# sid2364/dna-sequences-pg-extension

Hardware: AMD Instinct MI355X
Metric: k-mers/sec for k=31 count over 3 Gbase synthetic; % of HBM-read roofline (higher is better)
Workload: dtype u64; 1 GPU; config 4: k=31 count over 3000000000 synthetic bases (splitmix64 seed 0xd2a0003), unordered groups (super-k-mer partitioning), single GPU; n_bases=3000000000, k=31, distinct=2999999968

## Files before the change

dna-sequences-pg-extension_amd/csrc/kernels.hpp:

```cpp
#pragma once
#include <hip/hip_runtime.h>
#include <stdint.h>

#include "kmer_device.hpp"

namespace dnagpu {

hipError_t launch_synth(u64 *words, u64 w_begin, u64 w_end, u64 n_bases, u64 seed, u64 motif_len, hipStream_t s);
hipError_t launch_extract(const u64 *words, u64 n_words, u64 first, u64 count, int k, u64 *out_keys,
                          hipStream_t s);

constexpr int FILTER_MAX_GROUPS = 8192;
struct FilterSource {
    const u64 *words;
    u64 n_words;
    const u32 *marks;
    u64 n_mark_words;
    const u64 *seq_starts;
    u64 n_seqs;
};
void filter_bits_geometry(u64 count, u32 *n_groups, u32 *tiles_per_group);
hipError_t launch_filter_bits_count(const FilterSource &src, u64 first, u64 count, const FilterBits &fb, u32 *group_counts,
                                    hipStream_t s);
hipError_t launch_filter_bits_write(const FilterSource &src, u64 first, u64 count, const FilterBits &fb,
// ... 151 lines not shown
hipError_t launch_query_rank_scatter(const QHistSrc &s, u32 n_classes, u64 *cursors, u64 *out_keys, u64 *out_counts, u64 rows,
                                     hipStream_t st);
hipError_t launch_query_rank_scatter(const QAccSrc &s, u32 n_classes, u64 *cursors, u64 *out_keys, u64 *out_counts, u64 rows,
                                     hipStream_t st);
hipError_t launch_query_reverse(u64 *keys, u64 *counts, u64 n, hipStream_t st);

hipError_t launch_batch_marks(const u64 *starts, u64 n_seqs, u32 *marks, u64 n_mark_words, hipStream_t s);
hipError_t launch_batch_rows(const u64 *starts, u64 n_seqs, int k, u64 *rows, hipStream_t s);
hipError_t launch_batch_keys(const u64 *words, u64 n_words, const u32 *marks, u64 n_mark_words, u64 n_rows, int k, u64 *out_keys,
                             unsigned long long *cursor, hipStream_t s);

int sk_min_k();
int sk_minimizer_len(int k);
int sk_tile_rows();
int sk_max_c0();
hipError_t launch_sk_level0(bool scatter, const Chunk *chunks, u32 n_chunks, const u64 *words, u64 n_words, u64 first, int k,
                            u32 c0n, u32 b1bits, u32 r0bits, u32 *hist, const u32 *tot, void *recs, hipStream_t s,
                            u32 *aux = nullptr, const u32 *marks = nullptr, u64 n_mark_words = 0);
hipError_t launch_sk_sample_chunks(Chunk *chunks, u32 n_chunks, u32 stride, u32 len, u32 n, hipStream_t s);
int sk_slab_words();
u32 sk_slab_cap(u32 est, u64 chunk_rows, u64 sampled);
hipError_t launch_sk_slab_init(const u32 *est, u32 r0bits, u32 chunk_rows, u32 sampled, u32 n_chunks, u32 *slab, Node *nodes,
                               hipStream_t s);
hipError_t launch_sk_hist1(const Node *nodes, const Chunk *chunks, u32 n_chunks, const void *recs, u32 *hist, u32 *kcount,
                           hipStream_t s, bool by_d2 = false);
hipError_t launch_sk_scatter1(const Node *nodes, const Chunk *chunks, u32 n_chunks, const void *src, void *dst, const u32 *hist,
                              const u32 *tot, hipStream_t s, bool by_d2 = false, u32 *gcur = nullptr);
u64 sk_spec_span(u32 len, int bits);
hipError_t launch_sk_spec_regions(const Node *nodes, u32 n_nodes, u32 *spec, u32 *out, u32 *gcur, hipStream_t s,
                                  const u32 *rstart = nullptr);
hipError_t launch_sk_scatter1_spec(const Node *nodes, const Chunk *chunks, u32 n_chunks, const void *src, void *dst, u32 *gcur,
                                   const u32 *spec, u32 *kcount, u32 *over, hipStream_t s, const u32 *rstart = nullptr,
                                   const u32 *rcap = nullptr);
hipError_t launch_sk_spec_nodes(const Node *nodes, u32 n_nodes, const u32 *spec, const u32 *gcur, Node *next, u32 *over,
                                hipStream_t s, const u32 *rstart = nullptr, const u32 *rcap = nullptr);
u32 sk_sample1_len();
u32 sk_sample1_every();
hipError_t launch_sk_sampled_regions(const Node *nodes, const Chunk *samples, u32 n_samples, const void *recs, u32 n_mid, u32 *est,
                                     u32 *rcap, u32 *rstart, u32 *scan_tmp, u32 *total, hipStream_t s);
hipError_t launch_sk_heavy_finals(const Node *kids, u32 n, const u32 *kcount, Node *out, hipStream_t s);
int sk_flat_slice();
hipError_t launch_sk_take_heavy(Node *mids, const u32 *idx, u32 n_heavy, const u32 *kcount, Node *out, hipStream_t s);
hipError_t launch_sk_slice_count(const Node *buckets, u32 nb, u32 *n_slices, hipStream_t s);
hipError_t launch_sk_slice_fill(const Node *buckets, u32 nb, const u32 *slice_first, u32 *slice_rec0, u32 *slice_nrec, hipStream_t s);
hipError_t launch_sk_slice_kmers(const void *recs, const u32 *slice_rec0, const u32 *slice_nrec, u32 n_slices, u32 *slice_km,
                                 hipStream_t s);
hipError_t launch_sk_slice_nodes(const Node *buckets, u32 nb, const u32 *slice_first, const u32 *slice_koff, u32 n_slices,
                                 const u32 *total_keys, u32 key_base, int k, bool check_kmers, Node *out, u64 *n_bad, hipStream_t s);
hipError_t launch_sk_unmix(u64 *keys, u64 first, const u64 *end, u64 max_groups, int k, hipStream_t s);
hipError_t launch_sk_expand_flat(const void *recs, const u32 *slice_rec0, const u32 *slice_nrec, const u32 *slice_koff, u32 key_base,
                                 u32 n_slices, int k, u64 *keys, hipStream_t s);
int sk_regroup_tile();
hipError_t launch_sk_regroup(const Node *mids, u32 n_mids, const void *src, void *dst, Node *out_nodes, bool any_long, hipStream_t s);
hipError_t launch_sk_count(const Node *fin, const u32 *list, const u32 *list_off, u32 n_list, const void *recs, int k, u64 *n_groups,
                           u64 *seg_off, u32 *seg_cnt, u64 *out_keys, u32 *out_counts, u32 *left, hipStream_t s);

int sk_count_cap();
hipError_t launch_sk_select_flags(const Node *fin, u32 n_fin, u32 cap, u32 big_limit, u32 *f_small, u32 *f_big, u32 *k_range,
                                  u32 *k_big, hipStream_t s);
hipError_t launch_sk_select_lists(const Node *fin, u32 n_fin, u32 cap, u32 big_limit, const u32 *p_small, const u32 *p_big,
                                  const u32 *kb_range, u32 *list_small, u32 *off_small, u32 *list_big, u32 *off_big, hipStream_t s);
hipError_t launch_sk_over_flags(const Node *fin, u32 n_fin, u32 cap, u32 big_limit, const u32 *p_big, const u32 *big_status,
                                u32 *f_over, u32 *k_over, hipStream_t s);
hipError_t launch_sk_over_list(const Node *fin, u32 n_fin, const u32 *f_raw, const u32 *p_over, const u32 *kb_over, Node *over_nodes,
                               u32 *over_kbase, hipStream_t s);
hipError_t launch_sk_node_lens(const Node *nodes, u32 n, u32 *lens, hipStream_t s);
u32 sk_big_slice_records();
u64 sk_big_partial_slots();
hipError_t launch_sk_big_slices(const Node *fin, const u32 *list, u32 n_list, u32 *nsl, u32 *msl, hipStream_t s);
hipError_t launch_sk_big_slice_fill(const u32 *nsl_raw, const u32 *sfirst, u32 n_list, u32 *sl_bucket, u32 *sl_idx, hipStream_t s);
hipError_t launch_sk_count_big(const Node *fin, const u32 *list, const u32 *list_off, const u32 *nsl, const u32 *mfirst,
                               const u32 *sl_bucket, const u32 *sl_idx, u32 n_slices, u32 n_list, const void *recs, int k,
                               u64 *n_groups, u64 *seg_off, u32 *seg_cnt, u64 *out_keys, u32 *out_counts, u32 *status, u64 *part_keys,
                               u32 *part_cnts, u32 *part_n, bool any_sliced, hipStream_t s);

int scatter_tile_keys();
int scatter_threads();

}
```

dna-sequences-pg-extension_amd/csrc/sk_host.hip:

```cpp
#include "host_common.hpp"

using namespace dnagpu;


constexpr u64 SK_LEAF_MEAN = 2500;
constexpr u64 SK_MID_LIMIT = (u64)1 << 27;
#ifndef SK_MID_RECORDS_LOG2
#define SK_MID_RECORDS_LOG2 16
#endif
constexpr u32 SK_MID_RECORDS = 1u << SK_MID_RECORDS_LOG2;
constexpr u64 SK_BIG_LIMIT = 0xFFFFFFFFull;
constexpr int SK_B1_MAX = 9;
constexpr u64 SK_SLAB_MIN_ROWS = (u64)1 << 29;

template <typename T>
static int alloc1(PoolScope &ps, size_t n, T **out, size_t per = 1)
{
    return ps.alloc(std::max<size_t>(n, 1) * per, out);
}

static u32 sk_chunk_len(u64 x, u64 target = 4096, u64 tile = 8192)
{
    const u64 len = std::max<u64>(4 * tile, (x + target - 1) / target);
    return (u32)((len + tile - 1) / tile * tile);
// ... 476 lines not shown
    HIP_TRY(launch_level_children(hnodes, nh, lh.tot, lh.next, nullptr, nullptr, nullptr, 0, st));
    HIP_TRY(launch_sk_scatter1(hnodes, lh.chunks, lh.n_chunks, l1.rec1, p.rec0, lh.hist, lh.tot, st, true));
    p.heavy.total = 0;
    return DNAGPU_OK;
}

static int sk_level2(dnagpu_ctx *ctx, PoolScope &ps, SkParts &p, SkL1 &l1, const SkSplit &split)
{
    hipStream_t st = ctx->stream;
    const u32 n_mid = l1.lv.n_next, n_split = split.lv.n_next;
    Node *fn = nullptr;
    RC_TRY(ps.alloc((size_t)n_mid * 16 + n_split, &fn));
    prof_mark(ctx, "sk_regroup");
    bool any_long = false;
    for (u32 i = 0; i < n_mid && !any_long; i++)
        any_long = l1.rcn[i] > (u32)sk_regroup_tile();
    HIP_TRY(launch_sk_regroup(l1.lv.next, n_mid, l1.rec1, p.rec0, fn, any_long, st));
    if (n_split)
        HIP_TRY(launch_sk_heavy_finals(split.lv.next, n_split, split.kcount, fn + (size_t)n_mid * 16, st));
    if (!l1.rec1_kept)
        ps.free_now(l1.rec1);
    p.recs = p.rec0;
    p.fin = fn;
    p.n_fin = n_mid * 16 + n_split;
    return DNAGPU_OK;
}

static int sk_levels12(dnagpu_ctx *ctx, PoolScope &ps, SkParts &p)
{
    SkL1 l1;
    SkL1Route route;
    RC_TRY(sk_l1_plan(ctx, ps, p, l1));
    RC_TRY(sk_l1_route(ctx, ps, p, l1, &route));
    bool moved = false;
    if (route != SkL1Route::Exact)
        RC_TRY(sk_l1_speculative(ctx, ps, p, l1, route, &moved));
    if (!moved)
        RC_TRY(sk_l1_histogram(ctx, p, l1));
    std::vector<u32> heavy_idx;
    RC_TRY(sk_l1_census(ctx->debug_flags, l1, p, &heavy_idx));
    if (!moved)
        RC_TRY(sk_l1_scatter(ctx, ps, p, l1));
    SkSplit split;
    if (!heavy_idx.empty())
        RC_TRY(sk_heavy_take(ctx, ps, p, l1, heavy_idx, &split));
    return sk_level2(ctx, ps, p, l1, split);
}


struct SkTail {
    u32 *f_small = nullptr, *f_big = nullptr, *k_range = nullptr, *f_over = nullptr;
    u32 *scan_tmp = nullptr, *totals = nullptr;
    u32 *list_small = nullptr, *off_small = nullptr, *list_big = nullptr, *off_big = nullptr;
    u32 n_small = 0, n_big = 0, big_kmers = 0;
    u64 small_keys = 0;
    u64 out_cap = 0;
    u64 *cursor = nullptr;
    u64 *ok = nullptr;
    u32 *oc = nullptr;
    u64 *seg_off_fin = nullptr;
    u32 *seg_cnt_fin = nullptr;
    u32 *big_status = nullptr;
    Node *over_nodes = nullptr;
    u32 n_over = 0;
    u64 over_keys = 0;
    TreeResult tr = {};
    u64 *seg_off = nullptr;
    u32 *seg_cnt = nullptr;
    u32 n_segs = 0;
};

static int sk_tail_select(dnagpu_ctx *ctx, PoolScope &ps, const SkParts &p, u64 n, SkTail &t)
{
    hipStream_t st = ctx->stream;
    const u32 n_fin = p.n_fin;
    prof_mark(ctx, "sk_select");
    RC_TRY(ps.alloc((size_t)n_fin, &t.f_small));
    RC_TRY(ps.alloc((size_t)n_fin, &t.f_big));
    RC_TRY(ps.alloc((size_t)n_fin, &t.k_range));
    RC_TRY(ps.alloc((size_t)scan_tmp_words(n_fin) * 4, &t.scan_tmp));
    RC_TRY(ps.alloc(8, &t.totals));
    RC_TRY(ps.alloc((size_t)n_fin, &t.list_small));
    RC_TRY(ps.alloc((size_t)n_fin, &t.off_small));
    RC_TRY(ps.alloc((size_t)n_fin, &t.f_over));
    HIP_TRY(launch_sk_select_flags(p.fin, n_fin, (u32)sk_count_cap(), (u32)SK_BIG_LIMIT, t.f_small, t.f_big, t.k_range, t.f_over, st));
    HIP_TRY(launch_scan_u32_multi(scans_in_place({t.f_small, t.f_big, t.k_range, t.f_over}, t.totals, t.scan_tmp), 4, n_fin, st));
    u32 ht[4] = {0, 0, 0, 0};
    RC_TRY(read_back(ctx, ht, t.totals, sizeof ht));
    t.n_small = ht[0];
    t.n_big = ht[1];
    t.small_keys = ht[2];
    t.big_kmers = ht[3];
    t.out_cap = n + t.big_kmers;
    RC_TRY(alloc1(ps, t.n_big, &t.list_big));
    RC_TRY(alloc1(ps, t.n_big, &t.off_big));
    HIP_TRY(launch_sk_select_lists(p.fin, n_fin, (u32)sk_count_cap(), (u32)SK_BIG_LIMIT, t.f_small, t.f_big, t.k_range, t.list_small,
                                   t.off_small, t.list_big, t.off_big, st));
    return DNAGPU_OK;
}

static int sk_tail_outputs(dnagpu_ctx *ctx, PoolScope &ps, const SkParts &p, SkTail &t)
{
    hipStream_t st = ctx->stream;
    const u32 n_fin = p.n_fin;
    RC_TRY(ps.alloc(3, &t.cursor));
    RC_TRY(ps.alloc((size_t)t.out_cap, &t.ok));
    RC_TRY(ps.alloc((size_t)t.out_cap, &t.oc));
    const u64 init[3] = {t.small_keys, 0, 0};
    HIP_TRY(poke(t.cursor, init, sizeof init, st));
    RC_TRY(alloc1(ps, n_fin, &t.seg_off_fin));
    RC_TRY(alloc1(ps, n_fin, &t.seg_cnt_fin));
    HIP_TRY(hipMemsetAsync(t.seg_cnt_fin, 0, (size_t)n_fin * sizeof(u32), st));
    HIP_TRY(hipMemsetAsync(t.seg_off_fin, 0, (size_t)n_fin * sizeof(u64), st));
    RC_TRY(alloc1(ps, t.n_big, &t.big_status));
    return DNAGPU_OK;
}

static int sk_tail_count_big(dnagpu_ctx *ctx, PoolScope &ps, const SkParts &p, SkTail &t)
{
    hipStream_t st = ctx->stream;
    const u32 n_big = t.n_big;
    prof_mark(ctx, "sk_count_big");
    u32 *nsl = nullptr, *sfirst = nullptr, *mfirst = nullptr, *sl_bucket = nullptr, *sl_idx = nullptr, *part_n = nullptr, *part_cnts = nullptr;
    u64 *part_keys = nullptr;
    RC_TRY(ps.alloc((size_t)n_big, &nsl));
    RC_TRY(ps.alloc((size_t)n_big, &sfirst));
    RC_TRY(ps.alloc((size_t)n_big, &mfirst));
    HIP_TRY(launch_sk_big_slices(p.fin, t.list_big, n_big, nsl, mfirst, st));
    HIP_TRY(launch_scan_u32(nsl, sfirst, n_big, t.scan_tmp, t.totals + 6, st));
    HIP_TRY(launch_scan_u32(mfirst, mfirst, n_big, t.scan_tmp, t.totals + 7, st));
    u32 hs[2] = {0, 0};
    RC_TRY(read_back(ctx, hs, t.totals + 6, sizeof hs));
    const u32 n_slices = hs[0], n_part = hs[1];
    RC_TRY(alloc1(ps, n_slices, &sl_bucket));
    RC_TRY(alloc1(ps, n_slices, &sl_idx));
    RC_TRY(alloc1(ps, n_part, &part_n));
    RC_TRY(alloc1(ps, n_part, &part_keys, sk_big_partial_slots()));
    RC_TRY(alloc1(ps, n_part, &part_cnts, sk_big_partial_slots()));
    HIP_TRY(launch_sk_big_slice_fill(nsl, sfirst, n_big, sl_bucket, sl_idx, st));
    HIP_TRY(launch_sk_count_big(p.fin, t.list_big, t.off_big, nsl, mfirst, sl_bucket, sl_idx, n_slices, n_big, p.recs, p.k, t.cursor + 2,
                                t.seg_off_fin, t.seg_cnt_fin, t.ok, t.oc, t.big_status, part_keys, part_cnts, part_n, n_part > 0, st));
    return DNAGPU_OK;
}

static int sk_tail_select_over(dnagpu_ctx *ctx, PoolScope &ps, const SkParts &p, SkTail &t)
{
    hipStream_t st = ctx->stream;
    const u32 n_fin = p.n_fin;
    u32 *f_over_raw = nullptr, *k_over = nullptr, *over_kbase = nullptr;
    prof_mark(ctx, "sk_select_over");
// ... 43 lines not shown
        const u64 tree_keys = t.over_keys + heavy.total;
        if (tree_keys > 0xFFFFFFFFull)
            return DNAGPU_ERR_TOO_LARGE;
        const u32 n_tree = t.n_over + heavy.n;
        u64 *kbuf = nullptr;
        Node *knodes = nullptr;
        RC_TRY(ps.alloc((size_t)tree_keys, &kbuf));
        RC_TRY(ps.alloc((size_t)n_tree, &knodes));
        prof_mark(ctx, "sk_expand_flat");
        if (t.n_over)
            RC_TRY(sk_tail_expand(ctx, ps, t, p.k, t.over_nodes, t.n_over, p.recs, 0, true, kbuf, knodes));
        if (heavy.n)
            RC_TRY(sk_tail_expand(ctx, ps, t, p.k, heavy.nodes, heavy.n, heavy.recs, (u32)t.over_keys, heavy.counted, kbuf,
                                  knodes + t.n_over));
        RC_TRY(run_tree(ctx, ps, nullptr, 0, tree_keys, p.k, kbuf, 0, &t.tr, 0, 0, true, 0, ~0u, 0, knodes, n_tree, 2));
    }
#ifdef DNAGPU_STAMPS
    fprintf(stderr, "[sk select] n_fin %u small %u big %u (k-mers of big %u) over %u (keys %llu) heavy %u (keys %llu) tree nodes %u tiny %u small %u big %u\n",
            p.n_fin, t.n_small, t.n_big, t.big_kmers, t.n_over, (unsigned long long)t.over_keys, heavy.n,
            (unsigned long long)heavy.total, t.tr.n_nodes, t.tr.n_tiny, t.tr.n_small, t.tr.n_big);
#endif
    return DNAGPU_OK;
}

static int sk_tail_leaves(dnagpu_ctx *ctx, PoolScope &ps, const SkParts &p, SkTail &t)
{
    hipStream_t st = ctx->stream;
    const u32 n_fin = p.n_fin;
    const TreeResult &tr = t.tr;
    t.n_segs = n_fin + tr.n_nodes;
    RC_TRY(ps.alloc((size_t)t.n_segs, &t.seg_off));
    RC_TRY(ps.alloc((size_t)t.n_segs, &t.seg_cnt));
    HIP_TRY(hipMemcpyAsync(t.seg_cnt, t.seg_cnt_fin, (size_t)n_fin * sizeof(u32), hipMemcpyDeviceToDevice, st));
    HIP_TRY(hipMemcpyAsync(t.seg_off, t.seg_off_fin, (size_t)n_fin * sizeof(u64), hipMemcpyDeviceToDevice, st));
    if (tr.n_nodes > 0) {
        u32 *flags = nullptr, *ltmp = nullptr, *cls_list = nullptr;
        RC_TRY(ps.alloc((size_t)tr.n_nodes + 1, &flags));
        RC_TRY(ps.alloc((size_t)scan_tmp_words(tr.n_nodes), &ltmp));
        RC_TRY(ps.alloc((size_t)tr.n_nodes, &cls_list));
        prof_mark(ctx, "leaves");
        HIP_TRY(launch_leaves(tr.nodes, tr.n_nodes, tr.n_tiny, tr.n_small, tr.n_big, tr.buf0, tr.buf1, t.cursor, t.seg_off + n_fin,
                              t.seg_cnt + n_fin, t.ok, t.oc, flags, ltmp, cls_list, st, true, t.small_keys));
        HIP_TRY(launch_sk_unmix(t.ok, t.small_keys, t.cursor, tr.n_keys, p.k, st));
    }
    return DNAGPU_OK;
}

static int sk_tail_count(dnagpu_ctx *ctx, PoolScope &ps, const SkParts &p, SkTail &t)
{
    hipStream_t st = ctx->stream;
    prof_mark(ctx, "sk_count");
    u32 *left = nullptr;
    RC_TRY(ps.alloc((size_t)2 * t.n_small + 1, &left));
    HIP_TRY(launch_sk_count(p.fin, t.list_small, t.off_small, t.n_small, p.recs, p.k, t.cursor + 2, t.seg_off, t.seg_cnt, t.ok, t.oc, left,
                            st));
#ifdef DNAGPU_STAMPS
    {
        u32 nl = 0;
        RC_TRY(read_back(ctx, &nl, left + 2 * (size_t)t.n_small, 4));
        fprintf(stderr, "[sk count] %u small buckets, %u left to sk_count by sk_count_clean\n", t.n_small, nl);
    }
#endif
    return DNAGPU_OK;
}

static int sk_tail_finish(dnagpu_ctx *ctx, PoolScope &ps, const SkTail &t, u64 n, dnagpu_hist *h)
{
    prof_mark(ctx, "end");
    u64 fin_ctr[3] = {0, 0, 0};
    RC_TRY(read_back(ctx, fin_ctr, t.cursor, 24));
    const u64 extent = fin_ctr[0];
    const u64 total_groups = fin_ctr[2] + (extent - t.small_keys);
    if (fin_ctr[1] != 0) {
        set_err("super-k-mer count: %llu buckets whose records expand to a different number of k-mers than the partition counted",
                (unsigned long long)fin_ctr[1]);
        return DNAGPU_ERR_INTERNAL;
    }
    if (extent > t.out_cap) {
        set_err("super-k-mer count: %llu output slots used, %llu allocated", (unsigned long long)extent, (unsigned long long)t.out_cap);
        return DNAGPU_ERR_INTERNAL;
    }
    if (total_groups > n) {
        set_err("super-k-mer count: %llu groups for %llu rows", (unsigned long long)total_groups, (unsigned long long)n);
        return DNAGPU_ERR_INTERNAL;
    }
    h->total = n;
    hist_adopt(ps, h, t.ok, t.oc, t.seg_off, t.seg_cnt, t.n_segs, total_groups, false, extent);
    return DNAGPU_OK;
}

static int count_sk_tail(dnagpu_ctx *ctx, PoolScope &ps, const SkParts &p, u64 n, dnagpu_hist *h)
{
    SkTail t;
    RC_TRY(sk_tail_select(ctx, ps, p, n, t));
    RC_TRY(sk_tail_outputs(ctx, ps, p, t));
    if (t.n_big)
        RC_TRY(sk_tail_count_big(ctx, ps, p, t));
    RC_TRY(sk_tail_select_over(ctx, ps, p, t));
    RC_TRY(sk_tail_tree(ctx, ps, p, t));
    RC_TRY(sk_tail_leaves(ctx, ps, p, t));
    RC_TRY(sk_tail_count(ctx, ps, p, t));
    return sk_tail_finish(ctx, ps, t, n, h);
}

int dnagpu::count_sk(dnagpu_ctx *ctx, const SkRows &rows, int k, dnagpu_hist *h, u64 n_kmers_expected)
{
    PoolScope ps(ctx);
    SkParts p;
// ... 186 lines not shown
```

dna-sequences-pg-extension_amd/csrc/superkmer_kernels.hip:

```cpp
#include <algorithm>
#include <cstdlib>
#include <type_traits>

#include "kernels.hpp"

namespace dnagpu {

constexpr int SK_NT = 256;
constexpr int SKW_ROWS = 63 * 32;
constexpr int SK_TILE_ROWS = (SK_NT / 64) * SKW_ROWS;
constexpr int SK_MAX_C0 = 256;
constexpr int SKW_LIST = 768;
__host__ __device__ constexpr u32 sk_plain_max(int w) { return (u32)(2 * SKW_ROWS * 17 / (10 * (w + 1))) < (u32)SKW_LIST ? (u32)(2 * SKW_ROWS * 17 / (10 * (w + 1))) : (u32)SKW_LIST; }

int sk_tile_rows() { return SK_TILE_ROWS; }
int sk_max_c0() { return SK_MAX_C0; }
int sk_count_cap() { return 4096; }

typedef unsigned long long ull2_t __attribute__((ext_vector_type(2)));

constexpr int SK_REC_MULTI_BIT = 58;
constexpr int SK_POS_SHIFT = 39;
constexpr u32 SK_POS_MASK = 31u;
constexpr u32 SK_GPOS_MASK = 63u;
// ... 1740 lines not shown
                    ownq[q0 + q] = (unsigned short)((u32)tid | (q << 9));
            }
            myrec.x = myrec.y = 0;
            if (has_next2 && (u32)tid < nn2.len)
                myrec = recs[(u64)nn2.start + tid];
        }
        lq += step;
        li = ln;
        off = off_next;
        nd = nn;
        has_next = has_next2;
        ln = ln2;
        off_next = off2;
        nn = nn2;
    }
    emit_prev();
    if (tid == 0)
        atomicAdd(n_groups, (unsigned long long)my_groups);
}

__device__ __forceinline__ bool sk_records_share_kmer(const ull2_t A, u32 a, u32 nba, const ull2_t B, u32 b, u32 nbb, u32 m, u32 kmm)
{
    const u64 pm = ((u64)1 << 34) - 1;
    const u64 ah = A.y & pm, bh = B.y & pm;
    const u32 ML = a < b ? a : b;
    const u32 ra = nba - a - m, rb = nbb - b - m;
    const u32 MR = ra < rb ? ra : rb;
    const u64 xr = (sk_shr128(A.x, ah, 2u * (a + m)) ^ sk_shr128(B.x, bh, 2u * (b + m))) & (((u64)1 << (2u * MR)) - 1);
    const u32 R = xr ? (u32)__builtin_ctzll(xr) >> 1 : MR;
    if (R + ML < kmm)
        return false;
    const u64 xl = (funnel(A.x, ah, 2u * (a - ML)) ^ funnel(B.x, bh, 2u * (b - ML))) & (((u64)1 << (2u * ML)) - 1);
    const u32 L = xl ? ML - 1u - ((63u - (u32)__builtin_clzll(xl)) >> 1) : ML;
    return L + R >= kmm;
}


constexpr int SKQ_NT = 512;
static_assert(SKQ_NT == SKC_MAXREC, "a thread per record");
constexpr int SKQ_KMERS = 4096;
constexpr int SKQ_VSLOTS = 1024;
constexpr int SKQ_DIRTY_MAX = 640;

#if defined(SKQ_STORE_PLAIN) || defined(SKQ_KEYS_PLAIN)
#define SKQ_STORE(v, p) (*(p) = (v))
#else
#define SKQ_STORE(v, p) __builtin_nontemporal_store(v, p)
#endif
#if defined(SKQ_STORE_PLAIN) || defined(SKQ_COUNTS_PLAIN)
#define SKQ_STOREC(v, p) (*(p) = (v))
#else
#define SKQ_STOREC(v, p) __builtin_nontemporal_store(v, p)
#endif
__global__ __launch_bounds__(SKQ_NT, 8) void sk_count_clean_kernel(const Node *__restrict__ fin, const u32 *__restrict__ list,
                                                                   const u32 *__restrict__ list_off, u32 n_list,
                                                                   const ull2_t *__restrict__ recs, int k,
                                                                   unsigned long long *__restrict__ n_groups,
                                                                   u64 *__restrict__ seg_off, u32 *__restrict__ seg_cnt,
                                                                   u64 *__restrict__ out_keys, u32 *__restrict__ out_counts,
                                                                   u32 *__restrict__ left_list, u32 *__restrict__ left_off,
                                                                   u32 *__restrict__ n_left, int dbg)
{
    constexpr int WAVES = SKQ_NT / 64;
    __shared__ __attribute__((aligned(16))) ull2_t lrec[SKC_MAXREC];
    __shared__ __attribute__((aligned(16))) u64 vtab[SKQ_VSLOTS];
    __shared__ unsigned short own[SKQ_KMERS];
    __shared__ u32 wk[WAVES], wk2[WAVES];
    __shared__ u32 shared_flag[2], multi_flag[2];
    __shared__ u32 dcnt2[SKQ_VSLOTS / 2];
    __shared__ unsigned short cpos[SKC_MAXREC];
    __shared__ unsigned char rdb[SKC_MAXREC];
    __shared__ u32 d_ones;
    unsigned short *dcnt = reinterpret_cast<unsigned short *>(dcnt2);
    int tid = threadIdx.x;
    u32 lq = blockIdx.x;
    if (lq >= n_list)
        return;
    vtab[tid] = ~(u64)0;
    vtab[tid + SKQ_NT] = ~(u64)0;
    dcnt2[tid] = 0;
    rdb[tid] = 0;
    if (tid < 2)
        shared_flag[tid] = multi_flag[tid] = 0;
    if (tid == 0)
        d_ones = 0;
    const u32 mlen = k >= 23 ? 15u : (k >= 21 ? 13u : 12u);
    const u32 vmask = (1u << (2u * mlen)) - 1u, kmm = (u32)k - mlen;
    const u32 flank = kmm / 2u < 8u ? kmm / 2u : 8u, fmask = (1u << (2u * flank)) - 1u;
    const u32 hmask = (u32)(kmer_mask(k) >> 32);
    const u32 step = gridDim.x;
    u32 li = list[lq];
    Node nd = fin[li];
    ull2_t myrec;
    myrec.x = myrec.y = 0;
    if ((u32)tid < nd.len)
        myrec = recs[(u64)nd.start + tid];
    u64 my_groups = 0;
    int par = 0;
    for (;;) {
        const u32 off = list_off[lq];
        const bool has_next = lq + step < n_list;
        const u32 ln = has_next ? list[lq + step] : li;
        const Node nn = fin[ln];
        asm volatile("" : "+v"(tid));
        const int lane = tid & 63, wave = tid >> 6;
        const ull2_t me = myrec;
        lrec[tid] = me;
        myrec.x = myrec.y = 0;
        if (has_next && (u32)tid < nn.len)
            myrec = recs[(u64)nn.start + tid];
        const bool have = (u32)tid < nd.len;
        const u32 yh = (u32)(me.y >> 32);
        const u32 len = have ? ((yh >> 12) & 31u) + 1u : 0u;
        const u32 kinc = wave_incl_scan(len);
        if (lane == 63)
            wk[wave] = kinc;
        __syncthreads();
        u32 kbase = 0, n_km = 0;
        sk_wave_prefix16(wk, WAVES, wave, lane, kbase, n_km);
        u32 vslot = ~0u;
        if (have) {
            const u32 k0 = kbase + kinc - len;
            if (!SK_DBG(1024))
                for (u32 j = 0; j < len; j++)
                    own[k0 + j] = (unsigned short)((u32)tid | (j << 9));
            if (SK_DBG(256)) {
            } else if (yh & (1u << (SK_REC_MULTI_BIT - 32))) {
                multi_flag[par] = 1u;
            } else {
                const u32 p0 = (u32)me.x, p1 = (u32)(me.x >> 32), p2 = (u32)me.y, p3 = yh & 3u;
                const u32 a = (yh >> (SK_POS_SHIFT - 32)) & SK_POS_MASK;
                const u32 nba = len + (u32)k - 1u;
                const u32 sv = 2u * a, sl = 2u * (a - flank), sr = 2u * (a + mlen);
                const u32 v = __builtin_amdgcn_alignbit(sv >= 32u ? p2 : p1, sv >= 32u ? p1 : p0, sv) & vmask;
                u32 fl = __builtin_amdgcn_alignbit(sl >= 32u ? p2 : p1, sl >= 32u ? p1 : p0, sl) & fmask;
                const u32 r_lo = sr >= 64u ? p2 : (sr >= 32u ? p1 : p0), r_hi = sr >= 64u ? p3 : (sr >= 32u ? p2 : p1);
                u32 fr = __builtin_amdgcn_alignbit(r_hi, r_lo, sr) & fmask;
                const u32 mine_own = 0x8000u | (u32)tid;
                fl = a >= flank ? fl : mine_own;
                fr = nba - a - mlen >= flank ? fr : mine_own;
                const u32 hv = (v ^ (v >> 13)) * 0x85EBCA6Bu;
                const u32 lo32 = (hv >> 10) | ((u32)tid << 22), hi32 = fl | (fr << 16);
                const u64 mine = (u64)lo32 | ((u64)hi32 << 32);
                u32 slot = hv >> 22;
                for (;;) {
                    const u64 old = atomicCAS(reinterpret_cast<unsigned long long *>(&vtab[slot]), ~0ull, (unsigned long long)mine);
                    if (old == ~(u64)0)
                        break;
                    const u32 xl = (u32)old ^ lo32, xh = (u32)(old >> 32) ^ hi32;
                    if ((xl & 0x3FFFFFu) == 0 && ((xh & 0xFFFFu) == 0 || (xh >> 16) == 0)) {
                        const u32 oid = ((u32)old >> 22) & 511u;
                        const ull2_t ot = lrec[oid];
                        const u32 oyh = (u32)(ot.y >> 32);
                        if (sk_records_share_kmer(me, a, nba, ot, (oyh >> (SK_POS_SHIFT - 32)) & SK_POS_MASK,
                                                  ((oyh >> 12) & 31u) + (u32)k, mlen, kmm)) {
                            shared_flag[par] = 1u;
                            rdb[tid] = 1;
                            rdb[oid] = 1;
                        }
                    }
                    slot = (slot + 1u) & (u32)(SKQ_VSLOTS - 1);
                }
                vslot = slot;
            }
        }
        __syncthreads();
        if (vslot != ~0u)
            vtab[vslot] = ~(u64)0;
        u64 *ok = out_keys + off;
        u32 *oc = out_counts + off;
        auto key_cut = [&](const ull2_t r, u32 e) -> u64 {
            const u32 p0 = (u32)r.x, p1 = (u32)(r.x >> 32), p2 = (u32)r.y, p3 = (u32)(r.y >> 32) & 3u;
            const u32 sh = 2u * (e >> 9);
            const bool up = sh >= 32u;
            const u32 a0 = up ? p1 : p0, a1 = up ? p2 : p1, a2 = up ? p3 : p2;
            const u32 kl = __builtin_amdgcn_alignbit(a1, a0, sh), kh = __builtin_amdgcn_alignbit(a2, a1, sh) & hmask;
            return ((u64)kh << 32) | kl;
        };
        auto key_of = [&](u32 i) -> u64 {
            const u32 e = own[i];
            return key_cut(lrec[e & 511u], e);
        };
        const u32 flag = shared_flag[par] | (multi_flag[par] << 1);
        if (flag) {
            const bool dirty = have && rdb[tid] != 0;
            rdb[tid] = 0;
            const u32 pk = dirty ? (len << 16) : len;
            const u32 pinc = wave_incl_scan(pk);
            if (lane == 63)
                wk2[wave] = pinc;
            __syncthreads();
            u32 pbase = 0, ptot = 0;
            sk_wave_prefix16(wk2, WAVES, wave, lane, pbase, ptot);
            const u32 n_clean = ptot & 0xFFFFu, n_dirty = ptot >> 16;
            if ((flag & 2u) || n_dirty > (u32)SKQ_DIRTY_MAX) {
                if (tid == 0) {
                    const u32 d = atomicAdd(n_left, 1u);
                    left_list[d] = li;
                    left_off[d] = off;
                }
            } else {
                cpos[tid] = dirty ? (unsigned short)0xFFFFu : (unsigned short)((pbase + pinc - pk) & 0xFFFFu);
                __syncthreads();
                for (u32 i = (u32)tid; i < n_km; i += SKQ_NT) {
                    const u32 e = own[i];
                    const u32 c = cpos[e & 511u];
                    const u64 key = key_of(i);
                    if (c != 0xFFFFu) {
                        SKQ_STORE(key, &ok[c + (e >> 9)]);
                        SKQ_STOREC(1u, &oc[c + (e >> 9)]);
                    } else if (key == ~(u64)0) {
                        atomicAdd(&d_ones, 1u);
                    } else {
                        u32 slot = ((((u32)key ^ (u32)(key >> 32)) * 0x9E3779B1u) >> 22) & (u32)(SKQ_VSLOTS - 1);
                        for (;;) {
                            const u64 old = atomicCAS(reinterpret_cast<unsigned long long *>(&vtab[slot]), ~0ull, (unsigned long long)key);
                            if (old == ~(u64)0 || old == key)
                                break;
                            slot = (slot + 1u) & (u32)(SKQ_VSLOTS - 1);
                        }
                        atomicAdd(&dcnt2[slot >> 1], 1u << ((slot & 1u) * 16u));
// ... 43 lines not shown
            if ((u32)tid < head && (u32)tid < n_km) {
                SKQ_STORE(key_of((u32)tid), &ok[tid]);
                SKQ_STOREC(1u, &oc[tid]);
            }
            u32 i = head + 2u * (u32)tid;
            u32 e0 = 0, e1 = 0;
            ull2_t r0, r1;
            r0.x = r0.y = r1.x = r1.y = 0;
            auto fetch = [&](u32 at) {
                e0 = own[at];
                e1 = own[at + 1 < n_km ? at + 1 : at];
                asm volatile("" : "+v"(e0), "+v"(e1));
                r0 = lrec[e0 & 511u];
                r1 = lrec[e1 & 511u];
                asm volatile("" : "+v"(r0.x), "+v"(r0.y), "+v"(r1.x), "+v"(r1.y));
            };
            if (i < n_km)
                fetch(i);
            while (i < n_km) {
                const u32 ce0 = e0, ce1 = e1;
                const ull2_t c0 = r0, c1 = r1;
                const u32 nxt = i + 2u * SKQ_NT;
                if (nxt < n_km)
                    fetch(nxt);
                const u64 k0 = key_cut(c0, ce0);
                if (SK_DBG(512)) {
                    if (k0 == 0x123456789ull)
                        ok[0] = k0;
                } else if (i + 1 < n_km) {
                    ull2_t kk;
                    kk.x = k0;
                    kk.y = key_cut(c1, ce1);
                    SKQ_STORE(kk, reinterpret_cast<ull2_t *>(&ok[i]));
                    SKQ_STOREC((u64)0x100000001ull, reinterpret_cast<u64 *>(&oc[i]));
                } else {
                    SKQ_STORE(k0, &ok[i]);
                    SKQ_STOREC(1u, &oc[i]);
                }
                i = nxt;
            }
            if (tid == 0) {
                seg_off[li] = off;
                seg_cnt[li] = n_km;
                my_groups += n_km;
            }
        }
        if (tid == 0)
            shared_flag[par ^ 1] = multi_flag[par ^ 1] = 0;
        par ^= 1;
        if (!has_next)
            break;
        __syncthreads();
        lq += step;
        li = ln;
        nd = nn;
    }
    if (tid == 0 && my_groups)
        atomicAdd(n_groups, (unsigned long long)my_groups);
}

static int sk_dbg();

hipError_t launch_sk_count(const Node *fin, const u32 *list, const u32 *list_off, u32 n_list, const void *recs, int k, u64 *n_groups,
                           u64 *seg_off, u32 *seg_cnt, u64 *out_keys, u32 *out_counts, u32 *left ,
                           hipStream_t s)
{
    if (n_list == 0)
        return hipSuccess;
    int dev = 0, n_cu = 256, v = 0;
    if (hipGetDevice(&dev) == hipSuccess && hipDeviceGetAttribute(&v, hipDeviceAttributeMultiprocessorCount, dev) == hipSuccess && v > 0)
        n_cu = v;
    u32 *left_list = left, *left_off = left + n_list, *n_left = left + 2 * (size_t)n_list;
    hipError_t e = hipMemsetAsync(n_left, 0, sizeof(u32), s);
    if (e != hipSuccess)
        return e;
    hipLaunchKernelGGL(sk_count_clean_kernel, dim3(std::min<u32>(n_list, (u32)n_cu * 4u)), dim3(SKQ_NT), 0, s, fin, list, list_off, n_list,
                       reinterpret_cast<const ull2_t *>(recs), k, reinterpret_cast<unsigned long long *>(n_groups), seg_off, seg_cnt,
                       out_keys, out_counts, left_list, left_off, n_left, sk_dbg());
    const u32 grid = std::min<u32>(n_list, (u32)n_cu * 2u);
    hipLaunchKernelGGL(sk_count_kernel, dim3(grid), dim3(SKC_NT), 0, s, fin, left_list, left_off, 0u, n_left,
                       reinterpret_cast<const ull2_t *>(recs), k, reinterpret_cast<unsigned long long *>(n_groups), seg_off, seg_cnt,
                       out_keys, out_counts, sk_dbg());
    return hipGetLastError();
}

constexpr int SKB_NT = 1024;
constexpr int SKB_SLOTS = 8192;
constexpr int SKB_REC = 512;
constexpr int SKB_MAXQ = SKB_REC * 8;
constexpr u32 SKB_ROUND_CAP = SKB_SLOTS - SKB_NT * SKC_KPT - 64;
constexpr u64 SKB_EMPTY = ~(u64)0;
constexpr int SKB_RTAB_BITS = 10;
static_assert((1 << SKB_RTAB_BITS) == SKB_NT, "one record-table slot per thread");

__device__ __forceinline__ u32 skb_emit(const u64 *tab, const u32 *cnt, u32 n_ones, u32 *wtot, u64 *dst_keys, u32 *dst_counts)
{
    constexpr int WAVES = SKB_NT / 64;
    const int tid = threadIdx.x, lane = tid & 63, wave = tid >> 6;
    u64 myk[8];
    u32 myc[8], mine = 0;
#pragma unroll
    for (int j = 0; j < 8; j++) {
        myk[j] = tab[tid * 8 + j];
        myc[j] = cnt[tid * 8 + j];
        mine += myk[j] != SKB_EMPTY ? 1u : 0u;
    }
    const u32 inc = wave_incl_scan(mine);
    if (lane == 63)
        wtot[wave] = inc;
    __syncthreads();
    u32 before = 0, D = 0;
    sk_wave_prefix16(wtot, WAVES, wave, lane, before, D);
    u64 o = before + inc - mine;
#pragma unroll
    for (int j = 0; j < 8; j++)
        if (myk[j] != SKB_EMPTY) {
            dst_keys[o] = myk[j];
            dst_counts[o] = myc[j];
            o++;
        }
    if (n_ones && tid == 0) {
        dst_keys[D] = SKB_EMPTY;
        dst_counts[D] = n_ones;
    }
    return D + (n_ones ? 1u : 0u);
}

constexpr u32 SKB_SLICE_REC = 128 * SKB_REC;
constexpr u32 SKB_FAILED = ~0u;
// ... 322 lines not shown
        return hipSuccess;
    hipLaunchKernelGGL(sk_big_slice_fill_kernel, dim3((n_list + 3) / 4), dim3(256), 0, s, nsl_raw, sfirst, n_list, sl_bucket, sl_idx);
    return hipGetLastError();
}

hipError_t launch_sk_count_big(const Node *fin, const u32 *list, const u32 *list_off, const u32 *nsl, const u32 *mfirst,
                               const u32 *sl_bucket, const u32 *sl_idx, u32 n_slices, u32 n_list, const void *recs, int k,
                               u64 *n_groups, u64 *seg_off, u32 *seg_cnt, u64 *out_keys, u32 *out_counts, u32 *status, u64 *part_keys,
                               u32 *part_cnts, u32 *part_n, bool any_sliced, hipStream_t s)
{
    if (n_slices == 0)
        return hipSuccess;
    int dev = 0, n_cu = 256, v = 0;
    if (hipGetDevice(&dev) == hipSuccess && hipDeviceGetAttribute(&v, hipDeviceAttributeMultiprocessorCount, dev) == hipSuccess && v > 0)
        n_cu = v;
    const u32 grid = std::min<u32>(n_slices, (u32)n_cu);
    hipLaunchKernelGGL(sk_count_big_kernel, dim3(grid), dim3(SKB_NT), 0, s, fin, list, list_off, nsl, mfirst, sl_bucket, sl_idx,
                       n_slices, reinterpret_cast<const ull2_t *>(recs), k, reinterpret_cast<unsigned long long *>(n_groups), seg_off,
                       seg_cnt, out_keys, out_counts, status, part_keys, part_cnts, part_n);
    if (any_sliced)
        hipLaunchKernelGGL(sk_big_merge_kernel, dim3(n_list), dim3(SKB_NT), 0, s, fin, list, list_off, nsl, mfirst, n_list,
                           reinterpret_cast<unsigned long long *>(n_groups), seg_off, seg_cnt, out_keys, out_counts, status,
                           part_keys, part_cnts, part_n);
    return hipGetLastError();
}

__device__ __forceinline__ u32 sk_bucket_class(const Node &nd, u32 cap, u32 big_limit)
{
    const u32 km = nd.child_base;
    if (km == 0)
        return 0u;
    if (km <= cap && nd.len <= (u32)SKC_MAXREC && nd.chunk_base <= (u32)SKC_MAXQ)
        return 1u;
    return km > 2 * cap && km <= big_limit ? 2u : 3u;
}

__global__ __launch_bounds__(256) void sk_select_flags_kernel(const Node *__restrict__ fin, u32 n_fin, u32 cap, u32 big_limit,
                                                              u32 *__restrict__ f_small, u32 *__restrict__ f_big,
                                                              u32 *__restrict__ k_range, u32 *__restrict__ k_big)
{
    const u32 i = blockIdx.x * blockDim.x + threadIdx.x;
    if (i >= n_fin)
        return;
    const u32 c = sk_bucket_class(fin[i], cap, big_limit);
    f_small[i] = c == 1u ? 1u : 0u;
    f_big[i] = c == 2u ? 1u : 0u;
    k_range[i] = c == 1u || c == 2u ? fin[i].child_base : 0u;
    k_big[i] = c == 2u ? fin[i].child_base : 0u;
}

__global__ __launch_bounds__(256) void sk_select_lists_kernel(const Node *__restrict__ fin, u32 n_fin, u32 cap, u32 big_limit,
                                                              const u32 *__restrict__ p_small, const u32 *__restrict__ p_big,
                                                              const u32 *__restrict__ kb_range, u32 *__restrict__ list_small,
                                                              u32 *__restrict__ off_small, u32 *__restrict__ list_big,
                                                              u32 *__restrict__ off_big)
{
    const u32 i = blockIdx.x * blockDim.x + threadIdx.x;
    if (i >= n_fin)
        return;
    const u32 c = sk_bucket_class(fin[i], cap, big_limit);
    if (c == 1u) {
        list_small[p_small[i]] = i;
        off_small[p_small[i]] = kb_range[i];
    } else if (c == 2u) {
        list_big[p_big[i]] = i;
        off_big[p_big[i]] = kb_range[i];
    }
}

__global__ __launch_bounds__(256) void sk_over_flags_kernel(const Node *__restrict__ fin, u32 n_fin, u32 cap, u32 big_limit,
                                                            const u32 *__restrict__ p_big, const u32 *__restrict__ big_status,
                                                            u32 *__restrict__ f_over, u32 *__restrict__ k_over)
{
    const u32 i = blockIdx.x * blockDim.x + threadIdx.x;
    if (i >= n_fin)
        return;
    const u32 c = sk_bucket_class(fin[i], cap, big_limit);
    const bool over = c == 3u || (c == 2u && big_status[p_big[i]] != 0);
    f_over[i] = over ? 1u : 0u;
    k_over[i] = over ? fin[i].child_base : 0u;
}

__global__ __launch_bounds__(256) void sk_over_list_kernel(const Node *__restrict__ fin, u32 n_fin, const u32 *__restrict__ f_raw,
                                                           const u32 *__restrict__ p_over, const u32 *__restrict__ kb_over,
                                                           Node *__restrict__ over_nodes, u32 *__restrict__ over_kbase)
{
    const u32 i = blockIdx.x * blockDim.x + threadIdx.x;
    if (i >= n_fin || !f_raw[i])
        return;
    over_nodes[p_over[i]] = fin[i];
    over_kbase[p_over[i]] = kb_over[i];
}

hipError_t launch_sk_select_flags(const Node *fin, u32 n_fin, u32 cap, u32 big_limit, u32 *f_small, u32 *f_big, u32 *k_range,
                                  u32 *k_big, hipStream_t s)
{
    if (n_fin == 0)
        return hipSuccess;
    hipLaunchKernelGGL(sk_select_flags_kernel, dim3((n_fin + 255) / 256), dim3(256), 0, s, fin, n_fin, cap, big_limit, f_small, f_big,
                       k_range, k_big);
    return hipGetLastError();
}

hipError_t launch_sk_select_lists(const Node *fin, u32 n_fin, u32 cap, u32 big_limit, const u32 *p_small, const u32 *p_big,
                                  const u32 *kb_range, u32 *list_small, u32 *off_small, u32 *list_big, u32 *off_big, hipStream_t s)
{
    if (n_fin == 0)
        return hipSuccess;
    hipLaunchKernelGGL(sk_select_lists_kernel, dim3((n_fin + 255) / 256), dim3(256), 0, s, fin, n_fin, cap, big_limit, p_small, p_big,
                       kb_range, list_small, off_small, list_big, off_big);
    return hipGetLastError();
}

hipError_t launch_sk_over_flags(const Node *fin, u32 n_fin, u32 cap, u32 big_limit, const u32 *p_big, const u32 *big_status,
                                u32 *f_over, u32 *k_over, hipStream_t s)
{
    if (n_fin == 0)
        return hipSuccess;
    hipLaunchKernelGGL(sk_over_flags_kernel, dim3((n_fin + 255) / 256), dim3(256), 0, s, fin, n_fin, cap, big_limit, p_big, big_status,
                       f_over, k_over);
    return hipGetLastError();
}

hipError_t launch_sk_over_list(const Node *fin, u32 n_fin, const u32 *f_raw, const u32 *p_over, const u32 *kb_over, Node *over_nodes,
                               u32 *over_kbase, hipStream_t s)
{
    if (n_fin == 0)
        return hipSuccess;
    hipLaunchKernelGGL(sk_over_list_kernel, dim3((n_fin + 255) / 256), dim3(256), 0, s, fin, n_fin, f_raw, p_over, kb_over, over_nodes,
                       over_kbase);
    return hipGetLastError();
}

static int sk_dbg()
{
#ifdef DNAGPU_STAMPS
    const char *e = getenv("DNAGPU_DEBUG_SK");
    return e ? atoi(e) : 0;
#else
    return 0;
#endif
}

template <int W, bool BATCH>
static void launch_front(bool scatter, u32 n_chunks, hipStream_t s, const Chunk *chunks, const u64 *words, u64 n_words,
                         u64 first, int k, u32 lmax, u32 mmask, u32 c0n, u32 b1mask, u32 r0n, u32 *hist, const u32 *tot, void *recs,
                         u32 *aux, const u32 *marks, u64 n_mark_words)
{
    if (scatter)
        hipLaunchKernelGGL((sk_scatter0_kernel<W, BATCH>), dim3(n_chunks), dim3(SK_NT), 0, s, chunks, n_chunks, words, n_words, first,
                           k, lmax, mmask, c0n, b1mask, r0n, hist, tot, reinterpret_cast<ull2_t *>(recs), sk_dbg(), aux, marks,
                           n_mark_words);
    else
        hipLaunchKernelGGL((sk_hist0_kernel<W, BATCH>), dim3(n_chunks), dim3(SK_NT), 0, s, chunks, n_chunks, words, n_words, first,
                           lmax, mmask, c0n, b1mask, r0n, hist, aux, marks, n_mark_words);
}

int sk_min_k() { return 20; }
int sk_minimizer_len(int k) { return k >= 23 ? 15 : (k >= 21 ? 13 : 12); }

hipError_t launch_sk_level0(bool scatter, const Chunk *chunks, u32 n_chunks, const u64 *words, u64 n_words, u64 first, int k,
                            u32 c0n, u32 b1bits, u32 r0bits, u32 *hist, const u32 *tot, void *recs, hipStream_t s, u32 *aux,
                            const u32 *marks, u64 n_mark_words)
// ... 137 lines not shown
```

Before: 163.3 billion k-mers/s.

## Pack per-bucket descriptors and double-buffer records in sk_count_clean_kernel

```diff
diff --git a/dna-sequences-pg-extension_amd/csrc/kernels.hpp b/dna-sequences-pg-extension_amd/csrc/kernels.hpp
--- a/dna-sequences-pg-extension_amd/csrc/kernels.hpp
+++ b/dna-sequences-pg-extension_amd/csrc/kernels.hpp
@@ -227,14 +227,21 @@
                                  u32 n_slices, int k, u64 *keys, hipStream_t s);
 int sk_regroup_tile();
 hipError_t launch_sk_regroup(const Node *mids, u32 n_mids, const void *src, void *dst, Node *out_nodes, bool any_long, hipStream_t s);
-hipError_t launch_sk_count(const Node *fin, const u32 *list, const u32 *list_off, u32 n_list, const void *recs, int k, u64 *n_groups,
-                           u64 *seg_off, u32 *seg_cnt, u64 *out_keys, u32 *out_counts, u32 *left, hipStream_t s);
+struct alignas(16) SkItem {
+    u32 start;
+    u32 len;
+    u32 off;
+    u32 li;
+};
+hipError_t launch_sk_count(const Node *fin, const u32 *list, const u32 *list_off, const SkItem *items, u32 n_list, const void *recs, int k,
+                           u64 *n_groups, u64 *seg_off, u32 *seg_cnt, u64 *out_keys, u32 *out_counts, u32 *left, hipStream_t s);
 
 int sk_count_cap();
 hipError_t launch_sk_select_flags(const Node *fin, u32 n_fin, u32 cap, u32 big_limit, u32 *f_small, u32 *f_big, u32 *k_range,
                                   u32 *k_big, hipStream_t s);
 hipError_t launch_sk_select_lists(const Node *fin, u32 n_fin, u32 cap, u32 big_limit, const u32 *p_small, const u32 *p_big,
-                                  const u32 *kb_range, u32 *list_small, u32 *off_small, u32 *list_big, u32 *off_big, hipStream_t s);
+                                  const u32 *kb_range, u32 *list_small, u32 *off_small, SkItem *items_small, u32 *list_big, u32 *off_big,
+                                  hipStream_t s);
 hipError_t launch_sk_over_flags(const Node *fin, u32 n_fin, u32 cap, u32 big_limit, const u32 *p_big, const u32 *big_status,
                                 u32 *f_over, u32 *k_over, hipStream_t s);
 hipError_t launch_sk_over_list(const Node *fin, u32 n_fin, const u32 *f_raw, const u32 *p_over, const u32 *kb_over, Node *over_nodes,
diff --git a/dna-sequences-pg-extension_amd/csrc/sk_host.hip b/dna-sequences-pg-extension_amd/csrc/sk_host.hip
--- a/dna-sequences-pg-extension_amd/csrc/sk_host.hip
+++ b/dna-sequences-pg-extension_amd/csrc/sk_host.hip
@@ -552,6 +552,7 @@
     u32 *f_small = nullptr, *f_big = nullptr, *k_range = nullptr, *f_over = nullptr;
     u32 *scan_tmp = nullptr, *totals = nullptr;
     u32 *list_small = nullptr, *off_small = nullptr, *list_big = nullptr, *off_big = nullptr;
+    SkItem *items_small = nullptr;
     u32 n_small = 0, n_big = 0, big_kmers = 0;
     u64 small_keys = 0;
     u64 out_cap = 0;
@@ -594,8 +595,9 @@
     t.out_cap = n + t.big_kmers;
     RC_TRY(alloc1(ps, t.n_big, &t.list_big));
     RC_TRY(alloc1(ps, t.n_big, &t.off_big));
+    RC_TRY(alloc1(ps, t.n_small, &t.items_small));
     HIP_TRY(launch_sk_select_lists(p.fin, n_fin, (u32)sk_count_cap(), (u32)SK_BIG_LIMIT, t.f_small, t.f_big, t.k_range, t.list_small,
-                                   t.off_small, t.list_big, t.off_big, st));
+                                   t.off_small, t.items_small, t.list_big, t.off_big, st));
     return DNAGPU_OK;
 }
 
@@ -745,8 +747,8 @@
     prof_mark(ctx, "sk_count");
     u32 *left = nullptr;
     RC_TRY(ps.alloc((size_t)2 * t.n_small + 1, &left));
-    HIP_TRY(launch_sk_count(p.fin, t.list_small, t.off_small, t.n_small, p.recs, p.k, t.cursor + 2, t.seg_off, t.seg_cnt, t.ok, t.oc, left,
-                            st));
+    HIP_TRY(launch_sk_count(p.fin, t.list_small, t.off_small, t.items_small, t.n_small, p.recs, p.k, t.cursor + 2, t.seg_off, t.seg_cnt, t.ok,
+                            t.oc, left, st));
 #ifdef DNAGPU_STAMPS
     {
         u32 nl = 0;
diff --git a/dna-sequences-pg-extension_amd/csrc/superkmer_kernels.hip b/dna-sequences-pg-extension_amd/csrc/superkmer_kernels.hip
--- a/dna-sequences-pg-extension_amd/csrc/superkmer_kernels.hip
+++ b/dna-sequences-pg-extension_amd/csrc/superkmer_kernels.hip
@@ -1816,8 +1816,7 @@
 #else
 #define SKQ_STOREC(v, p) __builtin_nontemporal_store(v, p)
 #endif
-__global__ __launch_bounds__(SKQ_NT, 8) void sk_count_clean_kernel(const Node *__restrict__ fin, const u32 *__restrict__ list,
-                                                                   const u32 *__restrict__ list_off, u32 n_list,
+__global__ __launch_bounds__(SKQ_NT, 8) void sk_count_clean_kernel(const SkItem *__restrict__ items, u32 n_list,
                                                                    const ull2_t *__restrict__ recs, int k,
                                                                    unsigned long long *__restrict__ n_groups,
                                                                    u64 *__restrict__ seg_off, u32 *__restrict__ seg_cnt,
@@ -1826,7 +1825,7 @@
                                                                    u32 *__restrict__ n_left, int dbg)
 {
     constexpr int WAVES = SKQ_NT / 64;
-    __shared__ __attribute__((aligned(16))) ull2_t lrec[SKC_MAXREC];
+    __shared__ __attribute__((aligned(16))) ull2_t lrec2[2][SKC_MAXREC];
     __shared__ __attribute__((aligned(16))) u64 vtab[SKQ_VSLOTS];
     __shared__ unsigned short own[SKQ_KMERS];
     __shared__ u32 wk[WAVES], wk2[WAVES];
@@ -1853,33 +1852,40 @@
     const u32 flank = kmm / 2u < 8u ? kmm / 2u : 8u, fmask = (1u << (2u * flank)) - 1u;
     const u32 hmask = (u32)(kmer_mask(k) >> 32);
     const u32 step = gridDim.x;
-    u32 li = list[lq];
-    Node nd = fin[li];
-    ull2_t myrec;
-    myrec.x = myrec.y = 0;
-    if ((u32)tid < nd.len)
-        myrec = recs[(u64)nd.start + tid];
+    SkItem cur = items[lq];
+    bool has_next = lq + step < n_list;
+    SkItem nxt = items[has_next ? lq + step : lq];
+    ull2_t me;
+    me.x = me.y = 0;
+    if ((u32)tid < cur.len)
+        me = recs[(u64)cur.start + tid];
+    u32 kinc;
+    {
+        const u32 len0 = (u32)tid < cur.len ? (((u32)(me.y >> 32) >> 12) & 31u) + 1u : 0u;
+        kinc = wave_incl_scan(len0);
+        lrec2[0][tid] = me;
+        if ((tid & 63) == 63)
+            wk[tid >> 6] = kinc;
+    }
+    __syncthreads();
     u64 my_groups = 0;
     int par = 0;
     for (;;) {
-        const u32 off = list_off[lq];
-        const bool has_next = lq + step < n_list;
-        const u32 ln = has_next ? list[lq + step] : li;
-        const Node nn = fin[ln];
+        const bool has_next2 = (u64)lq + 2ull * step < n_list;
+        u32 ix2 = has_next2 ? lq + 2u * step : lq;
+        asm volatile("" : "+v"(ix2));
+        const SkItem nx2v = items[ix2];
+        const u32 off = cur.off, li = cur.li;
         asm volatile("" : "+v"(tid));
         const int lane = tid & 63, wave = tid >> 6;
-        const ull2_t me = myrec;
-        lrec[tid] = me;
+        const ull2_t *lrec = lrec2[par];
+        ull2_t myrec;
         myrec.x = myrec.y = 0;
-        if (has_next && (u32)tid < nn.len)
-            myrec = recs[(u64)nn.start + tid];
-        const bool have = (u32)tid < nd.len;
+        if (has_next && (u32)tid < nxt.len)
+            myrec = recs[(u64)nxt.start + tid];
+        const bool have = (u32)tid < cur.len;
         const u32 yh = (u32)(me.y >> 32);
         const u32 len = have ? ((yh >> 12) & 31u) + 1u : 0u;
-        const u32 kinc = wave_incl_scan(len);
-        if (lane == 63)
-            wk[wave] = kinc;
-        __syncthreads();
         u32 kbase = 0, n_km = 0;
         sk_wave_prefix16(wk, WAVES, wave, lane, kbase, n_km);
         u32 vslot = ~0u;
@@ -1931,6 +1937,16 @@
         __syncthreads();
         if (vslot != ~0u)
             vtab[vslot] = ~(u64)0;
+        SkItem nx2;
+        nx2.start = (u32)__builtin_amdgcn_readfirstlane((int)nx2v.start);
+        nx2.len = (u32)__builtin_amdgcn_readfirstlane((int)nx2v.len);
+        nx2.off = (u32)__builtin_amdgcn_readfirstlane((int)nx2v.off);
+        nx2.li = (u32)__builtin_amdgcn_readfirstlane((int)nx2v.li);
+        const u32 nlen = has_next && (u32)tid < nxt.len ? (((u32)(myrec.y >> 32) >> 12) & 31u) + 1u : 0u;
+        const u32 nkinc = wave_incl_scan(nlen);
+        lrec2[par ^ 1][tid] = myrec;
+        if (lane == 63)
+            wk[wave] = nkinc;
         u64 *ok = out_keys + off;
         u32 *oc = out_counts + off;
         auto key_cut = [&](const ull2_t r, u32 e) -> u64 {
@@ -2080,8 +2096,11 @@
             break;
         __syncthreads();
         lq += step;
-        li = ln;
-        nd = nn;
+        cur = nxt;
+        nxt = nx2;
+        has_next = has_next2;
+        me = myrec;
+        kinc = nkinc;
     }
     if (tid == 0 && my_groups)
         atomicAdd(n_groups, (unsigned long long)my_groups);
@@ -2089,8 +2108,8 @@
 
 static int sk_dbg();
 
-hipError_t launch_sk_count(const Node *fin, const u32 *list, const u32 *list_off, u32 n_list, const void *recs, int k, u64 *n_groups,
-                           u64 *seg_off, u32 *seg_cnt, u64 *out_keys, u32 *out_counts, u32 *left ,
+hipError_t launch_sk_count(const Node *fin, const u32 *list, const u32 *list_off, const SkItem *items, u32 n_list, const void *recs, int k,
+                           u64 *n_groups, u64 *seg_off, u32 *seg_cnt, u64 *out_keys, u32 *out_counts, u32 *left ,
                            hipStream_t s)
 {
     if (n_list == 0)
@@ -2102,7 +2121,7 @@
     hipError_t e = hipMemsetAsync(n_left, 0, sizeof(u32), s);
     if (e != hipSuccess)
         return e;
-    hipLaunchKernelGGL(sk_count_clean_kernel, dim3(std::min<u32>(n_list, (u32)n_cu * 4u)), dim3(SKQ_NT), 0, s, fin, list, list_off, n_list,
+    hipLaunchKernelGGL(sk_count_clean_kernel, dim3(std::min<u32>(n_list, (u32)n_cu * 4u)), dim3(SKQ_NT), 0, s, items, n_list,
                        reinterpret_cast<const ull2_t *>(recs), k, reinterpret_cast<unsigned long long *>(n_groups), seg_off, seg_cnt,
                        out_keys, out_counts, left_list, left_off, n_left, sk_dbg());
     const u32 grid = std::min<u32>(n_list, (u32)n_cu * 2u);
@@ -2531,8 +2550,8 @@
 __global__ __launch_bounds__(256) void sk_select_lists_kernel(const Node *__restrict__ fin, u32 n_fin, u32 cap, u32 big_limit,
                                                               const u32 *__restrict__ p_small, const u32 *__restrict__ p_big,
                                                               const u32 *__restrict__ kb_range, u32 *__restrict__ list_small,
-                                                              u32 *__restrict__ off_small, u32 *__restrict__ list_big,
-                                                              u32 *__restrict__ off_big)
+                                                              u32 *__restrict__ off_small, SkItem *__restrict__ items_small,
+                                                              u32 *__restrict__ list_big, u32 *__restrict__ off_big)
 {
     const u32 i = blockIdx.x * blockDim.x + threadIdx.x;
     if (i >= n_fin)
@@ -2541,6 +2560,12 @@
     if (c == 1u) {
         list_small[p_small[i]] = i;
         off_small[p_small[i]] = kb_range[i];
+        SkItem it;
+        it.start = fin[i].start;
+        it.len = fin[i].len;
+        it.off = kb_range[i];
+        it.li = i;
+        items_small[p_small[i]] = it;
     } else if (c == 2u) {
         list_big[p_big[i]] = i;
         off_big[p_big[i]] = kb_range[i];
@@ -2582,12 +2607,13 @@
 }
 
 hipError_t launch_sk_select_lists(const Node *fin, u32 n_fin, u32 cap, u32 big_limit, const u32 *p_small, const u32 *p_big,
-                                  const u32 *kb_range, u32 *list_small, u32 *off_small, u32 *list_big, u32 *off_big, hipStream_t s)
+                                  const u32 *kb_range, u32 *list_small, u32 *off_small, SkItem *items_small, u32 *list_big, u32 *off_big,
+                                  hipStream_t s)
 {
     if (n_fin == 0)
         return hipSuccess;
     hipLaunchKernelGGL(sk_select_lists_kernel, dim3((n_fin + 255) / 256), dim3(256), 0, s, fin, n_fin, cap, big_limit, p_small, p_big,
-                       kb_range, list_small, off_small, list_big, off_big);
+                       kb_range, list_small, off_small, items_small, list_big, off_big);
     return hipGetLastError();
 }
 
```

Result: no change. 164.4 billion k-mers/s, median of 6 (+0.7%).
